# intcomp/camouflaged-vlm

Hardware: AMD Instinct MI355X
Metric: images/sec at 1024x1024 (SAM-ViT-H + CLIP ViT-L/14), full cascade (higher is better)
Workload: dtype f16 hi.hi MFMA + block-scaled e4m3 MFMA for the two correction products (3 mantissa bits) in the ViT-H qkv / lin1 / lin2 and CLIP MLP GEMMs; 3x f16 split MFMA in the other GEMMs; f32 accumulate; ViT-H attention: q.k^T = ONE f16 product (Q and K as single f16 values), P.v = 2x f16 (P a single f16, V

## Files before the change

camouflaged-vlm_amd/csrc/attention_win2.hip:

```cpp
#include <stdlib.h>
#include <type_traits>
#include "common.h"
#include "../../include/cvlm.h"

namespace {

constexpr float LOG2E = 1.4426950408889634f;
typedef float f32x2 __attribute__((ext_vector_type(2)));

template <int OFF>
__device__ __forceinline__ half4 lds_read_tr16(unsigned lds_addr) {
    half4 r;
    asm volatile("ds_read_b64_tr_b16 %0, %1 offset:%2" : "=v"(r) : "v"(lds_addr), "n"(OFF));
    return r;
}
__device__ __forceinline__ void lds_wait() {
    asm volatile("s_waitcnt lgkmcnt(0)" ::: "memory");
    __builtin_amdgcn_sched_barrier(0);
}
template <int N> __device__ __forceinline__ void wait_vm() { asm volatile("s_waitcnt vmcnt(%0)" ::"n"(N) : "memory"); }
__device__ __forceinline__ void step_barrier() {
    asm volatile("s_waitcnt lgkmcnt(0)" ::: "memory");
    __builtin_amdgcn_s_barrier();
    asm volatile("" ::: "memory");
}

struct OneHotImage2 { half_t v[224 * 32]; };
constexpr OneHotImage2 make_onehot_image2() {
    OneHotImage2 im{};
    for (int s = 0; s < 224; ++s)
        for (int c = 0; c < 32; ++c) {
            const int kh = s / 14, kw = s % 14;
            const bool one = s < 196 && (c == kh || c == 16 + kw);
            const int chunk = (c >> 3) ^ ((s >> 2) & 3);
            im.v[s * 32 + chunk * 8 + (c & 7)] = one ? (half_t)1.0f : (half_t)0.0f;
        }
    return im;
}
__device__ const OneHotImage2 g_onehot2 = make_onehot_image2();

#ifdef CVLM_PROBES
__device__ unsigned long long* g_win2_trace = nullptr;
#define WIN2_STAMP(x) do { if (trace) { __builtin_amdgcn_sched_barrier(0); x = wall_clock64(); __builtin_amdgcn_sched_barrier(0); } } while (0)
#else
#define WIN2_STAMP(x) do { } while (0)
#endif

template <bool PLO, bool QLO, bool KLO>
__global__ __launch_bounds__(512, 1) void attn_win14p_kernel(const cvlm_attn_args g, const int nwx, const int npairs) {
    constexpr int HD = 80, KS = 5, NDB = 5, CPR = 10, KP = 80, VP = 80, L = 14, S_SEQ = 196;
    constexpr int KT = 32, NKT = 7, NCW = 7;
    constexpr int PLANE_B = 5120, SLOT_B = 2 * PLANE_B, IPP = 5;
    constexpr int OFF_K = 0, OFF_V = 3 * SLOT_B, OFF_T = 6 * SLOT_B;
    constexpr int RT_B = 27 * HD * 2, RS_PIECES = (4 * RT_B + 1023) / 1024, RS_B = RS_PIECES * 1024;
    constexpr int OFF_OH = OFF_T + RS_B, OH_B = 224 * 32 * 2;
    constexpr int OFF_TOK = OFF_OH + OH_B, TOK_B = 2 * 224 * 8;
    constexpr int TP = 17, OFF_TAUG = OFF_TOK + 2 * TOK_B;

    extern __shared__ __attribute__((aligned(16))) unsigned char smem[];
    const int tid = threadIdx.x, lane = tid & 63;
    const int wave = __builtin_amdgcn_readfirstlane(tid >> 6);
    const int qc = lane & 31, half = lane >> 5;
    const int D = g.heads * HD;
    const half_t* qkv_hi = (const half_t*)g.qkv_hi;
    const half_t* qkv_lo = (const half_t*)g.qkv_lo;
    const half_t* pad_hi = (const half_t*)g.pad_hi;
    const half_t* pad_lo = (const half_t*)g.pad_lo;
    const int64_t qkv_plane = qkv_lo - qkv_hi, pad_plane = pad_lo - pad_hi;
    const int nwin = nwx * nwx;
    const int SI = g.grid * g.grid;
    const QkvStrides QS = qkv_strides(g.qkv_layout, SI, g.B, g.heads, HD);
    const int my_items = blockIdx.x < npairs ? (npairs - 1 - (int)blockIdx.x) / (int)gridDim.x + 1 : 0;
    const int T = my_items * NKT;
    auto pair_of = [&](int k) -> int { return (int)blockIdx.x + k * (int)gridDim.x; };
    auto token_of = [&](int pair, int slot) -> int {
        const int seq = pair / g.heads;
        const int w = seq % nwin;
        const int wy = w / nwx, wx = w - wy * nwx;
        const int iy = slot / L, ix = slot - iy * L;
        const int y = wy * L + iy, x = wx * L + ix;
        if (y >= g.grid || x >= g.grid) return -1;
        return y * g.grid + x;
    };

    if (wave == NCW) {
        long long* tokoff = (long long*)(smem + OFF_TOK);
        auto fill_tokoff = [&](int k) {
            const int pair = pair_of(k);
            const int head = pair % g.heads, b = (pair / g.heads) / nwin;
            long long* tk = tokoff + (k & 1) * (TOK_B / 8);
            const long long pad_delta = pad_hi - qkv_hi;
#pragma unroll
            for (int r = 0; r < 4; ++r) {
                const int sl = lane + 64 * r;
                if (sl < 224) {
                    const int tok = token_of(pair, sl < S_SEQ ? sl : S_SEQ - 1);
                    const long long ko = tok < 0 ? pad_delta + D + head * HD : (long long)qkv_offset(QS, b, tok, 1, head);
                    tk[sl] = ko | (tok < 0 ? 1 : 0);
                    tk[224 + sl] = (ko + (tok < 0 ? (long long)D : (long long)QS.sop)) | (tok < 0 ? 1 : 0);
                }
            }
            asm volatile("s_waitcnt lgkmcnt(0)" ::: "memory");
        };
        int row_s[IPP], ch_s[IPP];
#pragma unroll
        for (int sub = 0; sub < IPP; ++sub) {
            const int c = sub * 64 + lane;
            row_s[sub] = c / CPR;
            ch_s[sub] = c - row_s[sub] * CPR;
        }
        auto issue_tile = [&](int op, int gt) {
            const int k = gt / NKT, t = gt - k * NKT;
            const long long* tk = tokoff + (k & 1) * (TOK_B / 8) + op * 224 + t * KT;
            unsigned char* dst = smem + (op ? OFF_V : OFF_K) + (gt % 3) * SLOT_B;
            const half_t* src[IPP][2];
#pragma unroll
            for (int sub = 0; sub < IPP; ++sub) {
                const long long ko = tk[row_s[sub]];
                const long long disp = (ko & 1) ? pad_plane : qkv_plane;
                src[sub][0] = qkv_hi + ((ko & ~7ll) + ch_s[sub] * 8);
                src[sub][1] = src[sub][0] + disp;
            }
#pragma unroll
            for (int pl = 0; pl < 2; ++pl) {
                if (!KLO && pl == 1 && op == 0) continue;
#pragma unroll
                for (int sub = 0; sub < IPP; ++sub) glds16(src[sub][pl], dst + pl * PLANE_B + sub * 1024);
            }
        };
        {
            const unsigned char* t0 = (const unsigned char*)g.relh_hi;
            const unsigned char* t1 = (const unsigned char*)g.relh_lo;
            const unsigned char* t2 = (const unsigned char*)g.relw_hi;
            const unsigned char* t3 = (const unsigned char*)g.relw_lo;
#pragma unroll 1
            for (int i = 0; i < RS_PIECES; ++i) {
                int byte = i * 1024 + lane * 16;
                if (byte >= 4 * RT_B) byte = 0;
                const int tbl = byte / RT_B, off = byte - tbl * RT_B;
                const unsigned char* src = (tbl == 0 ? t0 : (tbl == 1 ? t1 : (tbl == 2 ? t2 : t3))) + off;
                glds16(src, smem + OFF_T + i * 1024);
            }
            const unsigned char* oh = (const unsigned char*)g_onehot2.v;
#pragma unroll 1
            for (int i = 0; i < OH_B / 1024; ++i) glds16(oh + i * 1024 + lane * 16, smem + OFF_OH + i * 1024);
        }
        if (T > 0) {
            fill_tokoff(0);
            issue_tile(0, 0);
            if (T > 1) issue_tile(0, 1);
            if (T > 2) issue_tile(0, 2);
            issue_tile(1, 0);
            if (T > 1) issue_tile(1, 1);
        }
        wait_vm<0>();
        step_barrier();
#pragma unroll 1
        for (int gt = 0; gt < T; ++gt) {
            step_barrier();
            const int kn = gt + 3, vn = gt + 2;
            if (kn < T && kn % NKT == 0) fill_tokoff(kn / NKT);
#if defined(CVLM_WIN2_PROBE) && CVLM_WIN2_PROBE == 2
            const bool ik = false, iv = false;
#else
            const bool ik = kn < T, iv = vn < T;
#endif
            if (ik) issue_tile(0, kn);
            if (iv) issue_tile(1, vn);
            constexpr int KB = (KLO ? 2 : 1) * IPP, VB = 2 * IPP;
            if (ik && iv) wait_vm<KB + VB>();
            else if (ik) wait_vm<KB>();
            else if (iv) wait_vm<VB>();
            else wait_vm<0>();
        }
        return;
    }

    float* Taug = (float*)(smem + OFF_TAUG);
    const half_t* OH = (const half_t*)(smem + OFF_OH);
    auto k_slot = [&](int gt) -> const unsigned char* { return smem + OFF_K + (gt % 3) * SLOT_B; };
    auto v_slot = [&](int gt) -> const unsigned char* { return smem + OFF_V + (gt % 3) * SLOT_B; };
    const int tg = lane >> 4, ti = lane & 15;
    const int v_lane_off = (16 * (tg & 1) + 4 * (tg >> 1) + (ti >> 2)) * VP + 4 * (ti & 3);
    typedef std::integral_constant<bool, false> no_c;
    typedef std::integral_constant<bool, true> yes_c;
    bool first = true;
    const int qslot = wave * 32 + qc;
    const bool qvalid = qslot < S_SEQ;
    const int qs = qvalid ? qslot : S_SEQ - 1;
    half8 qn_h[KS], qn_l[KS];
    auto load_q = [&](int pair) {
        const int head = pair % g.heads, b = (pair / g.heads) / nwin;
        const int qtok = token_of(pair, qs);
        const int64_t qo = qtok < 0 ? (int64_t)head * HD : qkv_offset(QS, b, qtok, 0, head);
        const half_t* bh = (qtok < 0 ? pad_hi : qkv_hi) + qo;
        const half_t* bl = bh + (qtok < 0 ? pad_plane : qkv_plane);
#pragma unroll
        for (int ks = 0; ks < KS; ++ks) {
            qn_h[ks] = *(const half8*)(bh + 16 * ks + 8 * half);
            qn_l[ks] = *(const half8*)(bl + 16 * ks + 8 * half);
        }
    };
    if (my_items > 0) load_q(pair_of(0));
#ifdef CVLM_PROBES
    unsigned long long* const trace = g_win2_trace;
    unsigned long long ta = 0, tb = 0, tc = 0, td = 0, acc_u = 0, acc_t = 0, acc_o = 0, acc_bar = 0, t_first = 0;
#endif

#pragma unroll 1
    for (int k = 0; k < my_items; ++k) {
        const int pair = pair_of(k);
        const int head = pair % g.heads, b = (pair / g.heads) / nwin;
        const int gt0 = k * NKT;
        half8 qh[KS + 2], ql[KS + 2];
#pragma unroll
        for (int ks = 0; ks < KS; ++ks) { qh[ks] = qn_h[ks]; ql[ks] = qn_l[ks]; }
        if (first) { step_barrier(); first = false; }
        WIN2_STAMP(ta);
        {
            const int qhh = qs / L, qww = qs - qhh * L;
            float* Tq = Taug + (wave * 32 + qc) * TP;
            if (half == 0) { Tq[14] = 0.f; Tq[15] = 0.f; }
            const int rr = qc < 27 ? qc : 26;
            floatx16 u[2];
#pragma unroll
            for (int tb = 0; tb < 2; ++tb) {
                const unsigned char* rt = smem + OFF_T + (2 * tb) * RT_B + rr * (HD * 2) + 16 * half;
#pragma unroll
                for (int r = 0; r < 16; ++r) u[tb][r] = 0.f;
#pragma unroll
                for (int ks = 0; ks < KS; ++ks) {
                    const half8 rh = *(const half8*)(rt + 32 * ks);
                    const half8 rl = *(const half8*)(rt + RT_B + 32 * ks);
                    u[tb] = __builtin_amdgcn_mfma_f32_32x32x16_f16(rh, qh[ks], u[tb], 0, 0, 0);
                    u[tb] = __builtin_amdgcn_mfma_f32_32x32x16_f16(rl, qh[ks], u[tb], 0, 0, 0);
                    u[tb] = __builtin_amdgcn_mfma_f32_32x32x16_f16(rh, ql[ks], u[tb], 0, 0, 0);
                }
            }
            if (g.scale != 1.0f) {
#pragma unroll
                for (int ks = 0; ks < KS; ++ks)
#pragma unroll
                    for (int j = 0; j < 8; ++j) {
                        half_t hh, ll;
                        split_h2(((float)qh[ks][j] + (float)ql[ks][j]) * g.scale, hh, ll);
                        qh[ks][j] = hh;
                        ql[ks][j] = ll;
                    }
            }
#pragma unroll
            for (int tb = 0; tb < 2; ++tb) {
                int cq = tb ? qww : qhh;
                asm volatile("" : "+v"(cq), "+v"(u[tb][0]));
#pragma unroll
                for (int r = 0; r < 16; ++r) {
                    const int j = (r & 3) + 8 * (r >> 2) + 4 * half;
                    const int kidx = cq + L - 1 - j;
                    const bool ok = j < 27 && kidx >= 0 && kidx < L;
                    Tq[ok ? kidx : 16] = u[tb][r];
                }
                __builtin_amdgcn_wave_barrier();
                {
                    typedef unsigned u32x4_s __attribute__((ext_vector_type(4)));
                    u32x4_s h4, l4;
#pragma unroll
                    for (int j = 0; j < 4; ++j) {
                        unsigned a, b;
                        split_h2_pk(Tq[8 * half + 2 * j], Tq[8 * half + 2 * j + 1], a, b);
                        h4[j] = a; l4[j] = b;
                    }
                    qh[KS + tb] = __builtin_bit_cast(half8, h4);
                    ql[KS + tb] = __builtin_bit_cast(half8, l4);
                }
                __builtin_amdgcn_wave_barrier();
            }
        }

        WIN2_STAMP(tb);
        float m_run = -INFINITY, l_run = 0.f;
        floatx4 o[NDB][2];
#pragma unroll
        for (int n = 0; n < NDB; ++n)
#pragma unroll
            for (int qb = 0; qb < 2; ++qb) o[n][qb] = floatx4{0.f, 0.f, 0.f, 0.f};
        floatx4 osum[2] = {floatx4{0.f, 0.f, 0.f, 0.f}, floatx4{0.f, 0.f, 0.f, 0.f}};

        auto scores = [&](int t, auto last_c) -> floatx16 {
            floatx16 s;
#pragma unroll
            for (int r = 0; r < 16; ++r) s[r] = 0.f;
            const half_t* kr = (const half_t*)k_slot(gt0 + t) + qc * KP + 8 * half;
#pragma unroll
            for (int ks = 0; ks < KS; ++ks) {
                const half8 kh = *(const half8*)(kr + 16 * ks);
                s = __builtin_amdgcn_mfma_f32_32x32x16_f16(kh, qh[ks], s, 0, 0, 0);
                if constexpr (KLO) {
                    const half8 kl = *(const half8*)(kr + PLANE_B / 2 + 16 * ks);
                    s = __builtin_amdgcn_mfma_f32_32x32x16_f16(kl, qh[ks], s, 0, 0, 0);
                }
                if constexpr (QLO) s = __builtin_amdgcn_mfma_f32_32x32x16_f16(kh, ql[ks], s, 0, 0, 0);
            }
            const int row = t * KT + qc;
            const half_t* ohr = OH + row * 32;
#pragma unroll
            for (int a = 0; a < 2; ++a) {
                const half8 oh8 = *(const half8*)(ohr + 8 * ((half + 2 * a) ^ ((row >> 2) & 3)));
                s = __builtin_amdgcn_mfma_f32_32x32x16_f16(oh8, qh[KS + a], s, 0, 0, 0);
                s = __builtin_amdgcn_mfma_f32_32x32x16_f16(oh8, ql[KS + a], s, 0, 0, 0);
            }
            if (decltype(last_c)::value) {
                const int b0 = t * KT + 4 * half;
#pragma unroll
                for (int r = 0; r < 16; ++r)
                    if (b0 + (r & 3) + 8 * (r >> 2) >= S_SEQ) s[r] = -INFINITY;
            }
            return s;
        };
        floatx16 s_cur = scores(0, no_c{});

        auto tile = [&](int t, auto has_next_c, auto next_last_c) {
            constexpr bool HAS_NEXT = decltype(has_next_c)::value;
#ifdef CVLM_PROBES
            unsigned long long te = 0, tf = 0;
            WIN2_STAMP(te);
#endif
            step_barrier();
#ifdef CVLM_PROBES
            WIN2_STAMP(tf);
            if (trace) acc_bar += tf - te;
#endif
#if defined(CVLM_WIN2_PROBE) && CVLM_WIN2_PROBE == 1
            return;
#endif
            floatx16 s_next;
            if (HAS_NEXT) s_next = scores(t + 1, next_last_c);
            const unsigned vaddr = (unsigned)(size_t)(LDS_AS const unsigned char*)v_slot(gt0 + t) + 2u * (unsigned)v_lane_off;
            auto read_v = [&](auto db_c, half4 (&v0)[2], half4 (&v1)[2]) {
                constexpr int DB = decltype(db_c)::value;
                v0[0] = lds_read_tr16<2 * (16 * DB)>(vaddr);                 v1[0] = lds_read_tr16<2 * (16 * DB + 8 * VP)>(vaddr);
                v0[1] = lds_read_tr16<PLANE_B + 2 * (16 * DB)>(vaddr);       v1[1] = lds_read_tr16<PLANE_B + 2 * (16 * DB + 8 * VP)>(vaddr);
            };
            half4 va0[3][2], va1[3][2], vb0[2][2], vb1[2][2];
            read_v(std::integral_constant<int, 0>{}, va0[0], va1[0]);
            read_v(std::integral_constant<int, 1>{}, va0[1], va1[1]);
            read_v(std::integral_constant<int, 2>{}, va0[2], va1[2]);
            const floatx16 s = s_cur;
            float mx = fmaxf(s[0], s[1]);
#pragma unroll
            for (int r = 2; r < 16; r += 2) mx = fmaxf(fmaxf(mx, s[r]), s[r + 1]);
            mx = half_swap_max(mx);
            constexpr float TAU = 5.0f;
            if (__builtin_amdgcn_ballot_w64(mx > m_run + TAU) != 0) {
                const float m_new = fmaxf(m_run, mx);
                const float alpha = __builtin_amdgcn_exp2f((m_run - m_new) * LOG2E);
                l_run *= alpha;
                const auto ax = __builtin_amdgcn_permlane16_swap(__builtin_bit_cast(unsigned, alpha), __builtin_bit_cast(unsigned, alpha), false, false);
                const float a0 = __builtin_bit_cast(float, (unsigned)ax[0]), a1 = __builtin_bit_cast(float, (unsigned)ax[1]);
#pragma unroll
                for (int n = 0; n < NDB; ++n) { o[n][0] *= a0; o[n][1] *= a1; }
                osum[0] *= a0; osum[1] *= a1;
                m_run = m_new;
            }
            const f32x2 c2 = f32x2{-m_run * LOG2E, -m_run * LOG2E}, l2 = f32x2{LOG2E, LOG2E};
            f32x2 z[8], acc = f32x2{0.f, 0.f};
#pragma unroll
            for (int i = 0; i < 8; ++i) {
                const f32x2 a = f32x2{s[2 * i], s[2 * i + 1]} * l2 + c2;
                z[i] = f32x2{__builtin_amdgcn_exp2f(a.x), __builtin_amdgcn_exp2f(a.y)};
                acc += z[i];
            }
            l_run += acc.x + acc.y;
            typedef unsigned u32x4 __attribute__((ext_vector_type(4)));
            u32x4 xh[2], xl[2];
#pragma unroll
            for (int p2 = 0; p2 < 4; ++p2) {
                const f32x2 e0 = z[p2], e1 = z[4 + p2];
                unsigned h0, h1;
                if constexpr (PLO) {
                    h0 = __builtin_bit_cast(unsigned, __builtin_amdgcn_cvt_pkrtz(e0.x, e0.y));
                    h1 = __builtin_bit_cast(unsigned, __builtin_amdgcn_cvt_pkrtz(e1.x, e1.y));
                    const half2v f0 = __builtin_bit_cast(half2v, h0), f1 = __builtin_bit_cast(half2v, h1);
                    const unsigned l0 = __builtin_bit_cast(unsigned, __builtin_amdgcn_cvt_pkrtz(e0.x - (float)f0[0], e0.y - (float)f0[1]));
                    const unsigned l1 = __builtin_bit_cast(unsigned, __builtin_amdgcn_cvt_pkrtz(e1.x - (float)f1[0], e1.y - (float)f1[1]));
                    const auto rl = __builtin_amdgcn_permlane16_swap(l0, l1, false, false);
                    xl[0][p2] = (unsigned)rl[0]; xl[1][p2] = (unsigned)rl[1];
                } else {
                    h0 = __builtin_bit_cast(unsigned, __builtin_convertvector(e0, half2v));
                    h1 = __builtin_bit_cast(unsigned, __builtin_convertvector(e1, half2v));
                }
                const auto rh = __builtin_amdgcn_permlane16_swap(h0, h1, false, false);
                xh[0][p2] = (unsigned)rh[0]; xh[1][p2] = (unsigned)rh[1];
            }
            auto pv = [&](int db, half4 (&v0)[2], half4 (&v1)[2]) {
                const half8 vh = half8{v0[0][0], v0[0][1], v0[0][2], v0[0][3], v1[0][0], v1[0][1], v1[0][2], v1[0][3]};
                const half8 vl = half8{v0[1][0], v0[1][1], v0[1][2], v0[1][3], v1[1][0], v1[1][1], v1[1][2], v1[1][3]};
#pragma unroll
                for (int qb = 0; qb < 2; ++qb) {
                    const half8 bh = __builtin_bit_cast(half8, xh[qb]), bl = __builtin_bit_cast(half8, xl[qb]);
                    if (!PLO && db == 0) {
                        const half_t one = (half_t)1.0f;
                        osum[qb] = __builtin_amdgcn_mfma_f32_16x16x32_f16(half8{one, one, one, one, one, one, one, one}, bh, osum[qb], 0, 0, 0);
                    }
                    o[db][qb] = __builtin_amdgcn_mfma_f32_16x16x32_f16(vh, bh, o[db][qb], 0, 0, 0);
                    o[db][qb] = __builtin_amdgcn_mfma_f32_16x16x32_f16(vl, bh, o[db][qb], 0, 0, 0);
                    if constexpr (PLO) o[db][qb] = __builtin_amdgcn_mfma_f32_16x16x32_f16(vh, bl, o[db][qb], 0, 0, 0);
                }
            };
            lds_wait();
            read_v(std::integral_constant<int, 3>{}, vb0[0], vb1[0]);
            read_v(std::integral_constant<int, 4>{}, vb0[1], vb1[1]);
            pv(0, va0[0], va1[0]);
            pv(1, va0[1], va1[1]);
            pv(2, va0[2], va1[2]);
            lds_wait();
            pv(3, vb0[0], vb1[0]);
            pv(4, vb0[1], vb1[1]);
            if (HAS_NEXT) s_cur = s_next;
        };
#pragma unroll 1
        for (int t = 0; t < NKT - 2; ++t) tile(t, yes_c{}, no_c{});
        tile(NKT - 2, yes_c{}, yes_c{});
        if (k + 1 < my_items) load_q(pair_of(k + 1));
        tile(NKT - 1, no_c{}, no_c{});
        WIN2_STAMP(tc);

        float invq[2];
        if constexpr (PLO) {
            const float l_tot = half_swap_sum(l_run);
            const float inv = 1.0f / l_tot;
            const auto ix = __builtin_amdgcn_permlane16_swap(__builtin_bit_cast(unsigned, inv), __builtin_bit_cast(unsigned, inv), false, false);
            invq[0] = __builtin_bit_cast(float, (unsigned)ix[0]); invq[1] = __builtin_bit_cast(float, (unsigned)ix[1]);
        } else {
            invq[0] = 1.0f / osum[0][0]; invq[1] = 1.0f / osum[1][0];
        }
        const int g4 = lane >> 4;
#pragma unroll
        for (int qb = 0; qb < 2; ++qb) {
            const int qs2 = wave * 32 + 16 * qb + (lane & 15);
            const int tok2 = token_of(pair, qs2 < S_SEQ ? qs2 : S_SEQ - 1);
            const bool ok2 = qs2 < S_SEQ && tok2 >= 0;
            const int64_t orow = ((int64_t)b * SI + (ok2 ? tok2 : 0)) * D + head * HD;
            half_t* oh = (half_t*)g.out_hi + orow;
            half_t* ol = (half_t*)g.out_lo + orow;
            unsigned ph2[NDB][2][2];
#pragma unroll
            for (int n = 0; n < NDB; ++n) {
                split_h2_pk(o[n][qb][0] * invq[qb], o[n][qb][1] * invq[qb], ph2[n][0][0], ph2[n][1][0]);
                split_h2_pk(o[n][qb][2] * invq[qb], o[n][qb][3] * invq[qb], ph2[n][0][1], ph2[n][1][1]);
            }
#pragma unroll
            for (int pl = 0; pl < 2; ++pl) {
                half_t* dst = pl ? ol : oh;
#pragma unroll
                for (int pr = 0; pr < 2; ++pr) {
                    const auto r0 = __builtin_amdgcn_permlane16_swap(ph2[2 * pr][pl][0], ph2[2 * pr + 1][pl][0], false, false);
                    const auto r1 = __builtin_amdgcn_permlane16_swap(ph2[2 * pr][pl][1], ph2[2 * pr + 1][pl][1], false, false);
                    typedef unsigned u32x4 __attribute__((ext_vector_type(4)));
                    const u32x4 v = u32x4{(unsigned)r0[0], (unsigned)r1[0], (unsigned)r0[1], (unsigned)r1[1]};
                    const int d = (g4 & 1) ? 16 * (2 * pr + 1) + 4 * (g4 - 1) : 16 * (2 * pr) + 4 * g4;
                    if (ok2) *(u32x4*)(dst + d) = v;
                }
                typedef unsigned u32x2 __attribute__((ext_vector_type(2)));
                if (ok2) *(u32x2*)(dst + 64 + 4 * g4) = u32x2{ph2[4][pl][0], ph2[4][pl][1]};
            }
        }
#ifdef CVLM_PROBES
        WIN2_STAMP(td);
        if (trace) { acc_u += tb - ta; acc_t += tc - tb; acc_o += td - tc; if (k == 0) t_first = ta; }
#endif
    }
#ifdef CVLM_PROBES
    if (trace && lane == 0) {
        unsigned long long* o = trace + ((size_t)blockIdx.x * 8 + wave) * 8;
        o[0] = acc_u; o[1] = acc_t; o[2] = acc_o; o[3] = (unsigned long long)my_items; o[4] = t_first; o[5] = td; o[6] = acc_bar;
        o[7] = __builtin_amdgcn_s_getreg((31 << 11) | 4);
    }
#endif
    if (first) step_barrier();
}

}

#ifdef CVLM_PROBES
extern "C" int cvlm_debug_set_attn_win2_trace(void* buf) { return (int)hipMemcpyToSymbol(HIP_SYMBOL(g_win2_trace), &buf, sizeof(buf)); }
#endif

template <bool PLO, bool QLO, bool KLO>
static int launch_win14(const cvlm_attn_args& g, hipStream_t s) {
    constexpr int smem = 6 * 10240 + 17 * 1024 + 224 * 32 * 2 + 2 * (2 * 224 * 8) + 224 * 17 * 4;
    const int nwx = (g.grid + 13) / 14;
    const int npairs = g.heads * g.B * nwx * nwx;
    static bool attr[16] = {};
    if (cvlm_first_on_device(attr))
        (void)hipFuncSetAttribute((const void*)attn_win14p_kernel<PLO, QLO, KLO>, hipFuncAttributeMaxDynamicSharedMemorySize, smem);
    static int cus_[16] = {};
    int dev = 0;
    (void)hipGetDevice(&dev);
    int& cus = cus_[dev & 15];
    if (cus == 0 && hipDeviceGetAttribute(&cus, hipDeviceAttributeMultiprocessorCount, dev) != hipSuccess) cus = 256;
    const int wgs = npairs < cus ? npairs : cus;
    hipLaunchKernelGGL((attn_win14p_kernel<PLO, QLO, KLO>), dim3(wgs), dim3(512), smem, s, g, nwx, npairs);
    CVLM_CHECK_LAUNCH();
    return 0;
}

int cvlm_attention_window14_pc(const cvlm_attn_args& g, hipStream_t s) {
    if (g.split_qk == 3 && g.split_pv == 3) return launch_win14<true, true, true>(g, s);
    if (g.split_qk == 2 && g.split_pv == 2) return launch_win14<false, false, true>(g, s);
    if (g.split_qk == 1 && g.split_pv == 2) return launch_win14<false, false, false>(g, s);
    return CVLM_E_UNSUPPORTED;
}
```

camouflaged-vlm_amd/csrc/attention.hip:

```cpp
#include "common.h"
#include <stdlib.h>
#include "../../include/cvlm.h"

namespace {

constexpr float LOG2E = 1.4426950408889634f;
typedef float f32x2 __attribute__((ext_vector_type(2)));

struct AttnParams {
    cvlm_attn_args a;
    int S_seq;
    int L;
    int LTP;
    int nwx;
    int D;
};

__device__ __forceinline__ half4 lds_read_tr16(const half_t* p) {
    typedef __fp16 fp16x4 __attribute__((ext_vector_type(4)));
    fp16x4 r = __builtin_amdgcn_ds_read_tr16_b64_v4f16((LDS_AS fp16x4*)p);
    return __builtin_bit_cast(half4, r);
}

template <int HD, int NW, int MODE, int SQK, int SPV, bool CAUSAL>
// ... 177 lines not shown
                    const half8 kh = *(const half8*)(kr + 16 * ks);
                    s = __builtin_amdgcn_mfma_f32_32x32x16_f16(kh, qh[ks], s, 0, 0, 0);
                    if (SQK == 3) {
                        const half8 kl = *(const half8*)(kr + PLANE + 16 * ks);
                        s = __builtin_amdgcn_mfma_f32_32x32x16_f16(kl, qh[ks], s, 0, 0, 0);
                        s = __builtin_amdgcn_mfma_f32_32x32x16_f16(kh, ql[ks], s, 0, 0, 0);
                    }
                }
                const int b0 = t * 64 + sub * 32 + 4 * half;
                int kh0 = 0, kw0 = 0;
                if (MODE != 0) { kh0 = b0 / L; kw0 = b0 - kh0 * L; }
                float mx = -INFINITY;
                if (MODE == 0) {
                    if (CAUSAL || t * 64 + sub * 32 + 32 > S_seq) {
#pragma unroll
                        for (int r = 0; r < 16; ++r) {
                            const int slot = b0 + (r & 3) + 8 * (r >> 2);
                            const bool ok = (slot < S_seq) && (!CAUSAL || slot <= qslot);
                            s[r] = ok ? s[r] : -INFINITY;
                        }
                    }
#pragma unroll
                    for (int r = 0; r < 16; ++r) mx = fmaxf(mx, s[r]);
                    mx *= scale;
                }
#pragma unroll
                for (int r = 0; r < 16; ++r) {
                    if (MODE == 0) break;
                    const int c = (r & 3) + 8 * (r >> 2);
                    const int slot = b0 + c;
                    float v = s[r] * scale;
                    if (MODE != 0) {
                        int kw = kw0 + c, kh = kh0;
                        if (kw >= L) { kw -= L; ++kh; }
                        if (kw >= L) { kw -= L; ++kh; }
                        if (kw >= L) { kw -= L; ++kh; }
                        kh = kh < L ? kh : L - 1;
                        v += Thq[kh] + Twq[kw];
                    }
                    const bool ok = (slot < S_seq) && (!CAUSAL || slot <= qslot);
                    v = ok ? v : -INFINITY;
                    s[r] = v;
                    mx = fmaxf(mx, v);
                }
                mx = half_swap_max(mx);
                constexpr float TAU = 5.0f;
                if (__builtin_amdgcn_ballot_w64(mx > m_run + TAU) != 0) {
                    const float m_new = fmaxf(m_run, mx);
                    const float alpha = __builtin_amdgcn_exp2f((m_run - m_new) * LOG2E);
                    l_run *= alpha;
#pragma unroll
                    for (int n = 0; n < ND; ++n)
#pragma unroll
                        for (int r = 0; r < 16; ++r) o[n][r] *= alpha;
                    m_run = m_new;
                }
                const float lscale = MODE == 0 ? scale * LOG2E : LOG2E;
                const f32x2 c2 = f32x2{-m_run * LOG2E, -m_run * LOG2E}, l2 = f32x2{lscale, lscale};
                f32x2 z[8], acc = f32x2{0.f, 0.f};
#pragma unroll
                for (int i = 0; i < 8; ++i) {
                    const f32x2 a = f32x2{s[2 * i], s[2 * i + 1]} * l2 + c2;
                    z[i] = f32x2{__builtin_amdgcn_exp2f(a.x), __builtin_amdgcn_exp2f(a.y)};
                    acc += z[i];
                }
                l_run += acc.x + acc.y;
#pragma unroll
                for (int k2 = 0; k2 < 2; ++k2) {
                    half8 ph, pl;
#pragma unroll
                    for (int p2 = 0; p2 < 4; ++p2) {
                        const f32x2 e = z[4 * k2 + p2];
                        const half2v h = __builtin_bit_cast(half2v, __builtin_amdgcn_cvt_pkrtz(e.x, e.y));
                        ph[2 * p2] = h[0]; ph[2 * p2 + 1] = h[1];
                        if (SPV == 3) {
                            const half2v l = __builtin_bit_cast(half2v, split_lo_pk(__builtin_bit_cast(unsigned, h), e.x, e.y));
                            pl[2 * p2] = l[0]; pl[2 * p2 + 1] = l[1];
                        }
                    }
                    const half_t* vb = Vs + (sub * 32 + 16 * k2) * KP + v_lane_off;
#pragma unroll
                    for (int n = 0; n < ND; ++n) {
                        const half4 v0 = lds_read_tr16(vb + 32 * n);
                        const half4 v1 = lds_read_tr16(vb + 32 * n + 8 * KP);
                        const half8 vh = half8{v0[0], v0[1], v0[2], v0[3], v1[0], v1[1], v1[2], v1[3]};
                        o[n] = __builtin_amdgcn_mfma_f32_32x32x16_f16(vh, ph, o[n], 0, 0, 0);
                        if (SPV == 3) {
                            const half4 w0 = lds_read_tr16(vb + PLANE + 32 * n);
                            const half4 w1 = lds_read_tr16(vb + PLANE + 32 * n + 8 * KP);
                            const half8 vl = half8{w0[0], w0[1], w0[2], w0[3], w1[0], w1[1], w1[2], w1[3]};
                            o[n] = __builtin_amdgcn_mfma_f32_32x32x16_f16(vl, ph, o[n], 0, 0, 0);
                            o[n] = __builtin_amdgcn_mfma_f32_32x32x16_f16(vh, pl, o[n], 0, 0, 0);
                        }
                    }
                }
            }
        }
        __syncthreads();
    }

    const float l_tot = half_swap_sum(l_run);
    if (wave_active && qvalid && qtok >= 0) {
        const float inv = 1.0f / l_tot;
        const int64_t orow = ((int64_t)b * g.S + qtok) * D + head * HD;
        half_t* oh = (half_t*)g.out_hi + orow;
        half_t* ol = g.out_lo ? (half_t*)g.out_lo + orow : nullptr;
#pragma unroll
        for (int n = 0; n < ND; ++n)
#pragma unroll
            for (int rg = 0; rg < 4; ++rg) {
                const int d = 32 * n + 8 * rg + 4 * half;
                if (d < HD) {
                    half_t h[4], l4[4];
#pragma unroll
                    for (int j = 0; j < 4; ++j) split_h2(o[n][4 * rg + j] * inv, h[j], l4[j]);
                    *(half4*)(oh + d) = half4{h[0], h[1], h[2], h[3]};
                    if (ol) *(half4*)(ol + d) = half4{l4[0], l4[1], l4[2], l4[3]};
                }
            }
    }
}

template <int HD, int NW, int MODE, int SQK, int SPV, bool CAUSAL>
int launch(const AttnParams& p, hipStream_t s) {
    constexpr int KP = HD + 8;
    constexpr int NPL = (SQK == 3 || SPV == 3) ? 2 : 1;
    size_t smem = (size_t)2 * NPL * 64 * KP * 2 + 128 + 64 * 4;
    if (MODE != 0) smem += (size_t)2 * NW * 32 * p.LTP * 4;
    auto kern = attn_kernel<HD, NW, MODE, SQK, SPV, CAUSAL>;
    if (smem > 160 * 1024) return CVLM_E_UNSUPPORTED;
    if (smem > 48 * 1024)
        (void)hipFuncSetAttribute((const void*)kern, hipFuncAttributeMaxDynamicSharedMemorySize, (int)smem);
    const int nseq = (MODE == 2) ? p.a.B * p.nwx * p.nwx : p.a.B;
    const int q_rows = (MODE == 0 && p.a.q_rows > 0 && p.a.q_rows < p.S_seq) ? p.a.q_rows : p.S_seq;
    dim3 grid((q_rows + NW * 32 - 1) / (NW * 32), p.a.heads, nseq), block(NW * 64);
    hipLaunchKernelGGL(kern, grid, block, smem, s, p);
    CVLM_CHECK_LAUNCH();
    return 0;
}

template <int HD, int NW, int MODE, bool CAUSAL>
int launch_split(const AttnParams& p, hipStream_t s) {
    const int sq = p.a.split_qk, sp = p.a.split_pv;
    if ((sq == 3 && sp == 3) || (sq == 2 && sp == 2) || (sq == 1 && sp == 2)) return launch<HD, NW, MODE, 3, 3, CAUSAL>(p, s);
    if (sq == 3 && sp == 1) return launch<HD, NW, MODE, 3, 1, CAUSAL>(p, s);
    if (sq == 1 && sp == 1) return launch<HD, NW, MODE, 1, 1, CAUSAL>(p, s);
    return CVLM_E_UNSUPPORTED;
}

}

int cvlm_attention_global64_pp(const cvlm_attn_args& g, hipStream_t s);
int cvlm_attention_window14_pc(const cvlm_attn_args& g, hipStream_t s);

int64_t cvlm_attention_global64_pp_workspace_bytes(const cvlm_attn_args& g);

extern "C" int64_t cvlm_attention_workspace_bytes(const cvlm_attn_args* args) {
    if (!args) return 0;
    return cvlm_attention_global64_pp_workspace_bytes(*args);
}

extern "C" int cvlm_attention(const cvlm_attn_args* args, void* stream) {
    if (!args || !args->qkv_hi || !args->out_hi) return CVLM_E_BADARG;
    const cvlm_attn_args& g = *args;
    if (g.B <= 0 || g.S <= 0 || g.heads <= 0 || g.q_rows < 0 || (g.q_rows > 0 && g.mode != 0)) return CVLM_E_BADARG;
    if ((g.split_qk >= 2 || g.split_pv >= 2) && !g.qkv_lo) return CVLM_E_BADARG;
    AttnParams p;
    p.a = g;
    p.D = g.heads * g.hd;
    p.S_seq = g.S; p.L = 0; p.LTP = 0; p.nwx = 1;
    hipStream_t s = (hipStream_t)stream;
    if (g.mode == 0) {
        if (g.hd != 64) return CVLM_E_UNSUPPORTED;
        return g.causal ? launch_split<64, 4, 0, true>(p, s) : launch_split<64, 4, 0, false>(p, s);
    }
    if (g.hd != 80 || g.causal) return CVLM_E_UNSUPPORTED;
    if (!g.relh_hi || !g.relw_hi || (g.split_qk >= 2 && (!g.relh_lo || !g.relw_lo))) return CVLM_E_BADARG;
    if (g.grid <= 0 || g.S != g.grid * g.grid) return CVLM_E_BADARG;
    if (g.mode == 1) {
        const bool parity_split = (g.split_qk == g.split_pv && g.split_qk >= 2) || (g.split_qk == 1 && g.split_pv == 2);
        if ((g.grid == 64 || g.grid == 96) && parity_split) {
            const int rc = cvlm_attention_global64_pp(g, s);
            if (rc != CVLM_E_UNSUPPORTED) return rc;
        }
        p.L = g.grid; p.LTP = g.grid | 1;
        return launch_split<80, 4, 1, false>(p, s);
    }
    if (g.mode == 2) {
        if (g.window <= 0 || !g.pad_hi || ((g.split_qk >= 2 || g.split_pv >= 2) && !g.pad_lo)) return CVLM_E_BADARG;
        const bool parity_split = (g.split_qk == g.split_pv && g.split_qk >= 2) || (g.split_qk == 1 && g.split_pv == 2);
        if (g.window == 14 && parity_split && g.out_lo) return cvlm_attention_window14_pc(g, s);
        p.L = g.window; p.LTP = g.window | 1;
        p.nwx = (g.grid + g.window - 1) / g.window;
        p.S_seq = g.window * g.window;
        if (p.S_seq <= 7 * 32 && p.S_seq > 4 * 32) return launch_split<80, 7, 2, false>(p, s);
        return launch_split<80, 4, 2, false>(p, s);
    }
    return CVLM_E_BADARG;
}
```

Baseline: 64.71.

## Compact edge-window query slots and skip padded query waves in windowed attention

Query slots inside partial (edge) windows are now mapped compactly by the window's real row width, using a multiply-shift division that is checked at compile time. Waves whose query slots lie entirely in padding skip the compute and only take part in the barriers. Work items are also reordered so full windows are scheduled before edge and corner windows, to balance load across blocks. This trims wasted MFMA and softmax work on padded queries. The cost is extra per-pair index arithmetic and a barrier-only path that must stay in step with the producer wave.

```diff
diff --git a/camouflaged-vlm_amd/csrc/attention_win2.hip b/camouflaged-vlm_amd/csrc/attention_win2.hip
--- a/camouflaged-vlm_amd/csrc/attention_win2.hip
+++ b/camouflaged-vlm_amd/csrc/attention_win2.hip
@@ -45,6 +45,20 @@
 #else
 #define WIN2_STAMP(x) do { } while (0)
 #endif
+
+struct WinPair {
+    int b, head;
+    int tok0;
+    int rw, inv_rw;
+    int nreal;
+};
+constexpr bool win_slot_div_ok() {
+    for (int rw = 1; rw <= 14; ++rw)
+        for (int s = 0; s < 224; ++s)
+            if (((s * ((65536 + rw - 1) / rw)) >> 16) != s / rw) return false;
+    return true;
+}
+static_assert(win_slot_div_ok(), "slot -> window row by multiplication");
 
 template <bool PLO, bool QLO, bool KLO>
 __global__ __launch_bounds__(512, 1) void attn_win14p_kernel(const cvlm_attn_args g, const int nwx, const int npairs) {
@@ -72,7 +86,27 @@
     const QkvStrides QS = qkv_strides(g.qkv_layout, SI, g.B, g.heads, HD);
     const int my_items = blockIdx.x < npairs ? (npairs - 1 - (int)blockIdx.x) / (int)gridDim.x + 1 : 0;
     const int T = my_items * NKT;
-    auto pair_of = [&](int k) -> int { return (int)blockIdx.x + k * (int)gridDim.x; };
+    const int nfx = g.grid / L;
+    const int n_full = g.B * nfx * nfx * g.heads, n_edge = g.B * 2 * nfx * g.heads;
+    auto pair_of = [&](int k) -> int {
+        int p = (int)blockIdx.x + k * (int)gridDim.x;
+        if (nwx == nfx) return p;
+        int b, wy, wx, head;
+        if (p < n_full) {
+            const int q = p / g.heads, w = q % (nfx * nfx);
+            head = p - q * g.heads; b = q / (nfx * nfx);
+            wy = w / nfx; wx = w - wy * nfx;
+        } else if ((p -= n_full) < n_edge) {
+            const int q = p / g.heads, e = q % (2 * nfx);
+            head = p - q * g.heads; b = q / (2 * nfx);
+            wy = e < nfx ? e : nfx; wx = e < nfx ? nfx : e - nfx;
+        } else {
+            p -= n_edge;
+            b = p / g.heads; head = p - b * g.heads;
+            wy = nfx; wx = nfx;
+        }
+        return (b * nwin + wy * nwx + wx) * g.heads + head;
+    };
     auto token_of = [&](int pair, int slot) -> int {
         const int seq = pair / g.heads;
         const int w = seq % nwin;
@@ -186,15 +220,21 @@
     typedef std::integral_constant<bool, true> yes_c;
     bool first = true;
     const int qslot = wave * 32 + qc;
-    const bool qvalid = qslot < S_SEQ;
-    const int qs = qvalid ? qslot : S_SEQ - 1;
+    auto win_pair = [&](int pair) -> WinPair {
+        const int seq = pair / g.heads, b = seq / nwin, w = seq - b * nwin;
+        const int wy = w / nwx, wx = w - wy * nwx;
+        const int rh = min(L, g.grid - L * wy), rw = min(L, g.grid - L * wx);
+        return WinPair{b, pair - seq * g.heads, wy * L * g.grid + wx * L, rw, (65536 + rw - 1) / rw, rh * rw};
+    };
+    auto slot_row = [&](const WinPair& w, int s) -> int { return (s * w.inv_rw) >> 16; };
+    auto slot_tok = [&](const WinPair& w, int s, int row) -> int { return w.tok0 + row * g.grid + (s - row * w.rw); };
     half8 qn_h[KS], qn_l[KS];
     auto load_q = [&](int pair) {
-        const int head = pair % g.heads, b = (pair / g.heads) / nwin;
-        const int qtok = token_of(pair, qs);
-        const int64_t qo = qtok < 0 ? (int64_t)head * HD : qkv_offset(QS, b, qtok, 0, head);
-        const half_t* bh = (qtok < 0 ? pad_hi : qkv_hi) + qo;
-        const half_t* bl = bh + (qtok < 0 ? pad_plane : qkv_plane);
+        const WinPair wn = win_pair(pair);
+        if (wave * 32 >= wn.nreal) return;
+        const int qs = min(qslot, wn.nreal - 1);
+        const half_t* bh = qkv_hi + qkv_offset(QS, wn.b, slot_tok(wn, qs, slot_row(wn, qs)), 0, wn.head);
+        const half_t* bl = bh + qkv_plane;
 #pragma unroll
         for (int ks = 0; ks < KS; ++ks) {
             qn_h[ks] = *(const half8*)(bh + 16 * ks + 8 * half);
@@ -209,16 +249,24 @@
 
 #pragma unroll 1
     for (int k = 0; k < my_items; ++k) {
-        const int pair = pair_of(k);
-        const int head = pair % g.heads, b = (pair / g.heads) / nwin;
+        const WinPair wp = win_pair(pair_of(k));
         const int gt0 = k * NKT;
+        if (first) { step_barrier(); first = false; }
+        if (wave * 32 >= wp.nreal) {
+#pragma unroll 1
+            for (int t = 0; t < NKT - 1; ++t) step_barrier();
+            if (k + 1 < my_items) load_q(pair_of(k + 1));
+            step_barrier();
+            WIN2_STAMP(td);
+            continue;
+        }
         half8 qh[KS + 2], ql[KS + 2];
 #pragma unroll
         for (int ks = 0; ks < KS; ++ks) { qh[ks] = qn_h[ks]; ql[ks] = qn_l[ks]; }
-        if (first) { step_barrier(); first = false; }
         WIN2_STAMP(ta);
         {
-            const int qhh = qs / L, qww = qs - qhh * L;
+            const int qs = min(qslot, wp.nreal - 1);
+            const int qhh = slot_row(wp, qs), qww = qs - qhh * wp.rw;
             float* Tq = Taug + (wave * 32 + qc) * TP;
             if (half == 0) { Tq[14] = 0.f; Tq[15] = 0.f; }
             const int rr = qc < 27 ? qc : 26;
@@ -436,10 +484,12 @@
         const int g4 = lane >> 4;
 #pragma unroll
         for (int qb = 0; qb < 2; ++qb) {
+            if (wave * 32 + 16 * qb >= wp.nreal) continue;
             const int qs2 = wave * 32 + 16 * qb + (lane & 15);
-            const int tok2 = token_of(pair, qs2 < S_SEQ ? qs2 : S_SEQ - 1);
-            const bool ok2 = qs2 < S_SEQ && tok2 >= 0;
-            const int64_t orow = ((int64_t)b * SI + (ok2 ? tok2 : 0)) * D + head * HD;
+            const bool ok2 = qs2 < wp.nreal;
+            const int qs2c = ok2 ? qs2 : wp.nreal - 1;
+            const int tok2 = slot_tok(wp, qs2c, slot_row(wp, qs2c));
+            const int64_t orow = ((int64_t)wp.b * SI + tok2) * D + wp.head * HD;
             half_t* oh = (half_t*)g.out_hi + orow;
             half_t* ol = (half_t*)g.out_lo + orow;
             unsigned ph2[NDB][2][2];
```

New measurement: 64.72, median of 3. No clear change (+0.0%).

## Add dedicated pipelined CLIP attention kernel for head dim 64

Applied to the files above, without the earlier changes.

Adds a new non-causal hd=64 attention kernel for the CLIP path, enabled by default unless CVLM_ATTN_CLIP=0. It uses 512-thread workgroups in which two wave groups stream K and V tiles into a 4-slot LDS ring via direct global-to-LDS loads. Each workgroup covers up to eight 32-row query blocks, so K/V tiles are shared across more queries. It software-pipelines LDS reads against split f16 MFMAs and uses a lazy-rescale online softmax that only rescales when the max grows by more than a threshold. The aim is to cut K/V reload traffic and memory-latency stalls for CLIP attention, at the cost of heavy code complexity and tight barrier phasing.

```diff
diff --git a/camouflaged-vlm_amd/csrc/attention.hip b/camouflaged-vlm_amd/csrc/attention.hip
--- a/camouflaged-vlm_amd/csrc/attention.hip
+++ b/camouflaged-vlm_amd/csrc/attention.hip
@@ -353,6 +353,8 @@
 
 int cvlm_attention_global64_pp(const cvlm_attn_args& g, hipStream_t s);
 int cvlm_attention_window14_pc(const cvlm_attn_args& g, hipStream_t s);
+int cvlm_attention_clip(const cvlm_attn_args& g, hipStream_t s);
+bool cvlm_attention_clip_enabled();
 
 int64_t cvlm_attention_global64_pp_workspace_bytes(const cvlm_attn_args& g);
 
@@ -373,6 +375,10 @@
     hipStream_t s = (hipStream_t)stream;
     if (g.mode == 0) {
         if (g.hd != 64) return CVLM_E_UNSUPPORTED;
+        if (!g.causal && cvlm_attention_clip_enabled()) {
+            const int rc = cvlm_attention_clip(g, s);
+            if (rc != CVLM_E_UNSUPPORTED) return rc;
+        }
         return g.causal ? launch_split<64, 4, 0, true>(p, s) : launch_split<64, 4, 0, false>(p, s);
     }
     if (g.hd != 80 || g.causal) return CVLM_E_UNSUPPORTED;
diff --git a/camouflaged-vlm_amd/csrc/attention_clip.hip b/camouflaged-vlm_amd/csrc/attention_clip.hip
--- /dev/null
+++ b/camouflaged-vlm_amd/csrc/attention_clip.hip
@@ -0,0 +1,329 @@
+#include <stdlib.h>
+#include <string.h>
+#include <type_traits>
+#include <utility>
+#include "common.h"
+#include "../../include/cvlm.h"
+
+namespace {
+
+constexpr float LOG2E = 1.4426950408889634f;
+typedef float f32x2 __attribute__((ext_vector_type(2)));
+typedef unsigned u32x4 __attribute__((ext_vector_type(4)));
+
+template <int N> __device__ __forceinline__ void wait_vm() { asm volatile("s_waitcnt vmcnt(%0)" ::"n"(N) : "memory"); }
+__device__ __forceinline__ void phase_barrier() {
+    asm volatile("s_waitcnt lgkmcnt(0)" ::: "memory");
+    __builtin_amdgcn_s_barrier();
+    asm volatile("" ::: "memory");
+}
+
+constexpr int clip_reads(int J, int NPVS, int NST) {
+#ifdef CVLM_CLIP_PROBE_VB128
+    return J >= NST ? 0 : 2;
+#else
+    return J >= NST ? 0 : J < NPVS ? 4 : 2;
+#endif
+}
+template <class F, int... I> __device__ __forceinline__ void clip_for_each(F&& f, std::integer_sequence<int, I...>) {
+    (f(std::integral_constant<int, I>{}), ...);
+}
+
+constexpr int CLIP_HD = 64, CLIP_KT = 32, CLIP_KP = 72;
+constexpr int CLIP_PL_B = CLIP_KT * CLIP_KP * 2;
+constexpr int CLIP_SLOT_B = 2 * CLIP_PL_B;
+constexpr int CLIP_NSLOT = 4;
+constexpr int CLIP_SMEM = 2 * CLIP_NSLOT * CLIP_SLOT_B;
+
+__global__ __launch_bounds__(512, 2) void attn_clip_kernel(const cvlm_attn_args g, const int bpw, const int rows) {
+    constexpr int HD = CLIP_HD, KS = 4, NDB = 4, KT = CLIP_KT, KP = CLIP_KP, PL_B = CLIP_PL_B, SLOT_B = CLIP_SLOT_B;
+    constexpr int DPT = 3;
+
+    extern __shared__ __attribute__((aligned(16))) unsigned char smem[];
+    unsigned char* Kring = smem;
+    unsigned char* Vring = smem + CLIP_NSLOT * SLOT_B;
+
+    const int tid = threadIdx.x, lane = tid & 63;
+    const int wave = __builtin_amdgcn_readfirstlane(tid >> 6);
+    const bool grpB = wave >= 4;
+    const int qc = lane & 31, half = lane >> 5;
+    const int head = blockIdx.y, b = blockIdx.z;
+    const int S = g.S, D = g.heads * HD;
+    const int ntile = (S + KT - 1) / KT, npair = (ntile + 1) >> 1;
+    const half_t* qkv_hi = (const half_t*)g.qkv_hi;
+    const half_t* qkv_lo = (const half_t*)g.qkv_lo;
+    const QkvStrides QS = qkv_strides(g.qkv_layout, S, g.B, g.heads, HD);
+
+    const int cw = wave & 3;
+    const bool carrier = cw < 3;
+    const half_t* dsrc[DPT];
+    int drow[DPT];
+#pragma unroll
+    for (int j = 0; j < DPT; ++j) {
+        const int c = (cw * DPT + j) * 64 + lane;
+        const int pl = c >= 288 ? 1 : 0, cc = c - 288 * pl;
+        const int row = cc / 9;
+        int ch = cc - row * 9;
+        if (ch >= 8) ch = 0;
+        drow[j] = row & (KT - 1);
+        dsrc[j] = (pl ? qkv_lo : qkv_hi) + qkv_offset(QS, b, 0, grpB ? 2 : 1, head) + ch * 8;
+    }
+    int next_tile = 0;
+    auto issue_tile = [&](int slot) {
+        if (carrier && next_tile < ntile) {
+            unsigned char* base = (grpB ? Vring : Kring) + slot * SLOT_B + cw * DPT * 1024;
+#pragma unroll
+            for (int j = 0; j < DPT; ++j) {
+                int r = next_tile * KT + drow[j];
+                r = r < S ? r : S - 1;
+                glds16(dsrc[j] + (int64_t)r * QS.st, base + j * 1024);
+            }
+        }
+        ++next_tile;
+    };
+    issue_tile(0);
+    issue_tile(1);
+    if (!grpB) { issue_tile(2); issue_tile(3); }
+
+    const int jq = 2 * (wave & 3) + (wave >> 2);
+    const int q0 = (blockIdx.x * bpw + jq) * 32;
+    const bool active = jq < bpw && q0 < rows;
+    half8 qh[KS], ql[KS];
+    if (active) {
+        const int qslot = q0 + qc;
+        const int qs = qslot < S ? qslot : S - 1;
+        const int64_t qo = qkv_offset(QS, b, qs, 0, head);
+#pragma unroll
+        for (int ks = 0; ks < KS; ++ks) {
+            qh[ks] = *(const half8*)(qkv_hi + qo + 16 * ks + 8 * half);
+            ql[ks] = *(const half8*)(qkv_lo + qo + 16 * ks + 8 * half);
+        }
+    } else {
+#pragma unroll
+        for (int ks = 0; ks < KS; ++ks) { qh[ks] = half8{}; ql[ks] = half8{}; }
+    }
+
+    float m_run = -INFINITY, l_run = 0.f;
+    floatx16 s[2];
+    floatx4 o[NDB][2];
+#pragma unroll
+    for (int n = 0; n < NDB; ++n)
+#pragma unroll
+        for (int qb = 0; qb < 2; ++qb) o[n][qb] = floatx4{0.f, 0.f, 0.f, 0.f};
+#pragma unroll
+    for (int e = 0; e < 2; ++e)
+#pragma unroll
+        for (int r = 0; r < 16; ++r) s[e][r] = 0.f;
+    u32x4 xh[2][2] = {}, xl[2][2] = {};
+    const int k_lane_off = qc * KP + 8 * half;
+    const int tg = lane >> 4, ti = lane & 15;
+    const int v_lane_off = (16 * (tg & 1) + 4 * (tg >> 1) + (ti >> 2)) * KP + 4 * (ti & 3);
+    const float scale = g.scale;
+
+    auto Y = [&](auto npv_c, auto nqk_c, int vslot0, int kslot0) {
+        constexpr int NPV = decltype(npv_c)::value, NQK = decltype(nqk_c)::value;
+        constexpr int NPVS = NDB * NPV, NST = NPVS + KS * NQK, PD = 2, RS = PD + 1;
+        const unsigned va = (unsigned)(size_t)(LDS_AS const unsigned char*)(Vring + vslot0 * SLOT_B) + 2u * (unsigned)v_lane_off;
+        const unsigned ka = (unsigned)(size_t)(LDS_AS const unsigned char*)(Kring + kslot0 * SLOT_B) + 2u * (unsigned)k_lane_off;
+        half4 v0[RS][2], v1[RS][2];
+        half8 kf[RS][2];
+        auto load = [&](auto ic) {
+            constexpr int I = decltype(ic)::value;
+            const unsigned a_v = va, a_k = ka;
+            auto &kf_ = kf; auto &v0_ = v0; auto &v1_ = v1;
+            (void)a_v; (void)a_k; (void)kf_; (void)v0_; (void)v1_;
+            if constexpr (I < NPVS) {
+                constexpr int off = (I / NDB) * SLOT_B + 32 * (I % NDB);
+#ifdef CVLM_CLIP_PROBE_VB128
+                asm volatile("ds_read_b128 %0, %1 offset:%2" : "=v"(kf_[I % RS][0]) : "v"(a_k), "n"(off));
+                asm volatile("ds_read_b128 %0, %1 offset:%2" : "=v"(kf_[I % RS][1]) : "v"(a_k), "n"(off + PL_B));
+#else
+                asm volatile("ds_read_b64_tr_b16 %0, %1 offset:%2" : "=v"(v0_[I % RS][0]) : "v"(a_v), "n"(off));
+                asm volatile("ds_read_b64_tr_b16 %0, %1 offset:%2" : "=v"(v1_[I % RS][0]) : "v"(a_v), "n"(off + 16 * KP));
+                asm volatile("ds_read_b64_tr_b16 %0, %1 offset:%2" : "=v"(v0_[I % RS][1]) : "v"(a_v), "n"(off + PL_B));
+                asm volatile("ds_read_b64_tr_b16 %0, %1 offset:%2" : "=v"(v1_[I % RS][1]) : "v"(a_v), "n"(off + PL_B + 16 * KP));
+#endif
+            } else {
+                constexpr int off = ((I - NPVS) / KS) * SLOT_B + 32 * ((I - NPVS) % KS);
+                asm volatile("ds_read_b128 %0, %1 offset:%2" : "=v"(kf_[I % RS][0]) : "v"(a_k), "n"(off));
+                asm volatile("ds_read_b128 %0, %1 offset:%2" : "=v"(kf_[I % RS][1]) : "v"(a_k), "n"(off + PL_B));
+            }
+        };
+        auto compute = [&](auto ic) {
+            constexpr int I = decltype(ic)::value;
+            auto &kf_ = kf; auto &v0_ = v0; auto &v1_ = v1; auto &xh_ = xh; auto &xl_ = xl; auto &o_ = o; auto &s_ = s; auto &qh_ = qh; auto &ql_ = ql;
+            (void)kf_; (void)v0_; (void)v1_; (void)xh_; (void)xl_; (void)o_; (void)s_; (void)qh_; (void)ql_;
+            if constexpr (I < NPVS) {
+                constexpr int e = I / NDB, db = I % NDB;
+#ifdef CVLM_CLIP_PROBE_VB128
+                const half8 vh = kf_[I % RS][0], vl = kf_[I % RS][1];
+#else
+                const half4 a0 = v0_[I % RS][0], a1 = v1_[I % RS][0], b0 = v0_[I % RS][1], b1 = v1_[I % RS][1];
+                const half8 vh = half8{a0[0], a0[1], a0[2], a0[3], a1[0], a1[1], a1[2], a1[3]};
+                const half8 vl = half8{b0[0], b0[1], b0[2], b0[3], b1[0], b1[1], b1[2], b1[3]};
+#endif
+#pragma unroll
+                for (int qb = 0; qb < 2; ++qb) {
+                    const half8 bh = __builtin_bit_cast(half8, xh_[e][qb]), bl = __builtin_bit_cast(half8, xl_[e][qb]);
+                    o_[db][qb] = __builtin_amdgcn_mfma_f32_16x16x32_f16(vh, bh, o_[db][qb], 0, 0, 0);
+                    o_[db][qb] = __builtin_amdgcn_mfma_f32_16x16x32_f16(vl, bh, o_[db][qb], 0, 0, 0);
+                    o_[db][qb] = __builtin_amdgcn_mfma_f32_16x16x32_f16(vh, bl, o_[db][qb], 0, 0, 0);
+                }
+            } else {
+                constexpr int e = (I - NPVS) / KS, ks = (I - NPVS) % KS;
+                const half8 kh = kf_[I % RS][0], kl = kf_[I % RS][1];
+                if constexpr (ks == 0) {
+#pragma unroll
+                    for (int r = 0; r < 16; ++r) s_[e][r] = 0.f;
+                }
+                s_[e] = __builtin_amdgcn_mfma_f32_32x32x16_f16(kh, qh_[ks], s_[e], 0, 0, 0);
+                s_[e] = __builtin_amdgcn_mfma_f32_32x32x16_f16(kl, qh_[ks], s_[e], 0, 0, 0);
+                s_[e] = __builtin_amdgcn_mfma_f32_32x32x16_f16(kh, ql_[ks], s_[e], 0, 0, 0);
+            }
+        };
+        load(std::integral_constant<int, 0>{});
+        if constexpr (NST > 1) load(std::integral_constant<int, 1>{});
+        auto stage = [&](auto ic) {
+            constexpr int I = decltype(ic)::value;
+            if constexpr (I + PD < NST) load(std::integral_constant<int, I + PD>{});
+            constexpr int younger = clip_reads(I + 1, NPVS, NST) + clip_reads(I + 2, NPVS, NST);
+            asm volatile("s_waitcnt lgkmcnt(%0)" ::"n"(younger) : "memory");
+            __builtin_amdgcn_sched_barrier(0);
+            compute(ic);
+            __builtin_amdgcn_sched_barrier(0);
+        };
+        clip_for_each(stage, std::make_integer_sequence<int, NST>{});
+    };
+    typedef std::integral_constant<int, 0> n0_c;
+    typedef std::integral_constant<int, 1> n1_c;
+    typedef std::integral_constant<int, 2> n2_c;
+    auto X = [&](int p) {
+#pragma unroll
+        for (int e = 0; e < 2; ++e) {
+            const int t0 = (2 * p + e) * KT;
+            if (t0 + KT > S) {
+                const int b0 = t0 + 4 * half;
+#pragma unroll
+                for (int r = 0; r < 16; ++r) s[e][r] = (b0 + (r & 3) + 8 * (r >> 2) < S) ? s[e][r] : -INFINITY;
+            }
+        }
+        float mx0 = fmaxf(s[0][0], s[0][1]), mx1 = fmaxf(s[1][0], s[1][1]);
+#pragma unroll
+        for (int r = 2; r < 16; r += 2) {
+            mx0 = fmaxf(fmaxf(mx0, s[0][r]), s[0][r + 1]);
+            mx1 = fmaxf(fmaxf(mx1, s[1][r]), s[1][r + 1]);
+        }
+        const float mx = half_swap_max(fmaxf(mx0, mx1) * scale);
+        constexpr float TAU = 5.0f;
+        if (__builtin_amdgcn_ballot_w64(mx > m_run + TAU) != 0) {
+            const float m_new = fmaxf(m_run, mx);
+            const float alpha = __builtin_amdgcn_exp2f((m_run - m_new) * LOG2E);
+            l_run *= alpha;
+            const auto ax = __builtin_amdgcn_permlane16_swap(__builtin_bit_cast(unsigned, alpha), __builtin_bit_cast(unsigned, alpha), false, false);
+            const float a0 = __builtin_bit_cast(float, (unsigned)ax[0]), a1 = __builtin_bit_cast(float, (unsigned)ax[1]);
+#pragma unroll
+            for (int n = 0; n < NDB; ++n) { o[n][0] *= a0; o[n][1] *= a1; }
+            m_run = m_new;
+        }
+        const f32x2 c2 = f32x2{-m_run * LOG2E, -m_run * LOG2E}, l2 = f32x2{scale * LOG2E, scale * LOG2E};
+        f32x2 acc0 = f32x2{0.f, 0.f}, acc1 = f32x2{0.f, 0.f};
+        f32x2 z[2][8];
+#pragma unroll
+        for (int i = 0; i < 8; ++i) {
+            const f32x2 a0 = f32x2{s[0][2 * i], s[0][2 * i + 1]} * l2 + c2, a1 = f32x2{s[1][2 * i], s[1][2 * i + 1]} * l2 + c2;
+            z[0][i] = f32x2{__builtin_amdgcn_exp2f(a0.x), __builtin_amdgcn_exp2f(a0.y)};
+            z[1][i] = f32x2{__builtin_amdgcn_exp2f(a1.x), __builtin_amdgcn_exp2f(a1.y)};
+            acc0 += z[0][i];
+            acc1 += z[1][i];
+        }
+        l_run += (acc0.x + acc0.y) + (acc1.x + acc1.y);
+#pragma unroll
+        for (int e = 0; e < 2; ++e)
+#pragma unroll
+            for (int p2 = 0; p2 < 4; ++p2) {
+                const f32x2 v0 = z[e][p2], v1 = z[e][4 + p2];
+                const unsigned h0 = __builtin_bit_cast(unsigned, __builtin_amdgcn_cvt_pkrtz(v0.x, v0.y));
+                const unsigned h1 = __builtin_bit_cast(unsigned, __builtin_amdgcn_cvt_pkrtz(v1.x, v1.y));
+                const unsigned l0 = split_lo_pk(h0, v0.x, v0.y);
+                const unsigned l1 = split_lo_pk(h1, v1.x, v1.y);
+                const auto rl = __builtin_amdgcn_permlane16_swap(l0, l1, false, false);
+                xl[e][0][p2] = (unsigned)rl[0]; xl[e][1][p2] = (unsigned)rl[1];
+                const auto rh = __builtin_amdgcn_permlane16_swap(h0, h1, false, false);
+                xh[e][0][p2] = (unsigned)rh[0]; xh[e][1][p2] = (unsigned)rh[1];
+            }
+    };
+
+    wait_vm<0>();
+    phase_barrier();
+    if (grpB) phase_barrier();
+    if (active) {
+        if (ntile >= 2) Y(n0_c{}, n2_c{}, 0, 0);
+        else Y(n0_c{}, n1_c{}, 0, 0);
+    }
+    phase_barrier();
+#pragma unroll 1
+    for (int p = 0; p < npair; ++p) {
+        const int cur = 2 * (p & 1), oth = 2 - cur;
+        if (grpB && p + 1 < npair) { issue_tile(oth); issue_tile(oth + 1); }
+        if (active) X(p);
+        if (!grpB) wait_vm<0>();
+        phase_barrier();
+        if (!grpB && p + 2 < npair) { issue_tile(cur); issue_tile(cur + 1); }
+        if (active) {
+            const int nq = ntile - 2 * (p + 1);
+            if (nq >= 2) Y(n2_c{}, n2_c{}, cur, oth);
+            else if (nq == 1) Y(n2_c{}, n1_c{}, cur, oth);
+            else if (ntile - 2 * p >= 2) Y(n2_c{}, n0_c{}, cur, oth);
+            else Y(n1_c{}, n0_c{}, cur, oth);
+        }
+        if (grpB) wait_vm<0>();
+        phase_barrier();
+    }
+    if (!grpB) phase_barrier();
+
+    if (!active) return;
+    const float l_tot = half_swap_sum(l_run);
+    const float inv = 1.0f / l_tot;
+    const auto ix = __builtin_amdgcn_permlane16_swap(__builtin_bit_cast(unsigned, inv), __builtin_bit_cast(unsigned, inv), false, false);
+    const float invq[2] = {__builtin_bit_cast(float, (unsigned)ix[0]), __builtin_bit_cast(float, (unsigned)ix[1])};
+#pragma unroll
+    for (int qb = 0; qb < 2; ++qb) {
+        const int qs2 = q0 + 16 * qb + (lane & 15);
+        if (qs2 >= rows) continue;
+        const int64_t orow = ((int64_t)b * S + qs2) * D + head * HD + 4 * (lane >> 4);
+        half_t* oh = (half_t*)g.out_hi + orow;
+        half_t* ol = g.out_lo ? (half_t*)g.out_lo + orow : nullptr;
+#pragma unroll
+        for (int n = 0; n < NDB; ++n) {
+            half_t h[4], l4[4];
+#pragma unroll
+            for (int j = 0; j < 4; ++j) split_h2(o[n][qb][j] * invq[qb], h[j], l4[j]);
+            *(half4*)(oh + 16 * n) = half4{h[0], h[1], h[2], h[3]};
+            if (ol) *(half4*)(ol + 16 * n) = half4{l4[0], l4[1], l4[2], l4[3]};
+        }
+    }
+}
+
+}
+
+bool cvlm_attention_clip_enabled() {
+    const char* e = getenv("CVLM_ATTN_CLIP");
+    return !(e && e[0] == '0' && e[1] == '\0');
+}
+
+int cvlm_attention_clip(const cvlm_attn_args& g, hipStream_t s) {
+    const bool splits = (g.split_qk == 3 && g.split_pv == 3) || (g.split_qk == 2 && g.split_pv == 2) || (g.split_qk == 1 && g.split_pv == 2);
+    if (g.mode != 0 || g.hd != CLIP_HD || g.causal || !splits || !g.qkv_lo) return CVLM_E_UNSUPPORTED;
+    const int S = g.S;
+    const int nblk = (S + 31) / 32, nwg = (nblk + 7) / 8, bpw = (nblk + nwg - 1) / nwg;
+    const int q = (g.q_rows > 0 && g.q_rows < S) ? g.q_rows : S;
+    const int r128 = (q + 127) / 128 * 128;
+    const int rows = r128 < S ? r128 : S;
+    const int gx = ((rows + 31) / 32 + bpw - 1) / bpw;
+    static bool attr[16] = {};
+    if (cvlm_first_on_device(attr))
+        (void)hipFuncSetAttribute((const void*)attn_clip_kernel, hipFuncAttributeMaxDynamicSharedMemorySize, CLIP_SMEM);
+    hipLaunchKernelGGL(attn_clip_kernel, dim3(gx, g.heads, g.B), dim3(512), CLIP_SMEM, s, g, bpw, rows);
+    CVLM_CHECK_LAUNCH();
+    return 0;
+}
```

Result: no change. 65.51 before, 65.44 after (median of 2 runs) (-0.1%).
